# gam0022/hanamaru-renderer

Hardware: AMD Instinct MI355X
Metric: Mpaths/sec at 1920x1080x1024spp (rtcamp6 scene); achieved GB/s in BVH traversal (higher is better)
Workload: dtype f32

## Files before the change

hanamaru-renderer_amd/csrc/device_scene.h:

```cpp
#pragma once
#include <math.h>
#include <stdint.h>

#if defined(__HIPCC__)
#define HD __host__ __device__ __forceinline__
#else
#define HD inline
#endif

namespace hr {

struct alignas(16) f4 { float x, y, z, w; };

struct alignas(16) Node {
    float nearx, neary, farx, fary;
    float nearz, farz;
    uint32_t a;
    uint32_t b;
};
HD void node_set_box(Node &n, const float *mn, const float *mx, int octant) {
    n.nearx = (octant & 1) ? mx[0] : mn[0]; n.farx = (octant & 1) ? mn[0] : mx[0];
    n.neary = (octant & 2) ? mx[1] : mn[1]; n.fary = (octant & 2) ? mn[1] : mx[1];
    n.nearz = (octant & 4) ? mx[2] : mn[2]; n.farz = (octant & 4) ? mn[2] : mx[2];
}
// ... 156 lines not shown
    return B;
}
HD uint32_t gov_producer_prio(int32_t level, uint32_t init_prio) { return level <= 0 ? (init_prio | init_prio << 2) : level == 1 ? init_prio : 0u; }

struct RenderParams {
    uint32_t width, height;
    uint32_t tiles_x, tiles_y;
    uint32_t sampling_begin, stride, num_k;
    uint32_t adv_den;
    uint32_t leaf_den;
    uint32_t pad[3];
    uint32_t trace_boost;
    uint32_t node_unroll;
    uint32_t kchunk;
    uint32_t ovf_cap;
    uint32_t rr_start;
    uint32_t gov_slot;
    uint32_t nee_cull_off;
    uint32_t tail_div;
    uint32_t wg_budget;
    GovDev *gov;
    uint64_t rec_lo_off;
    uint32_t org_x, org_y, reg_w, reg_h;
};
HD uint32_t rp_reg_w(const RenderParams &rp) { return rp.reg_w ? rp.reg_w : rp.width; }
HD uint32_t rp_reg_h(const RenderParams &rp) { return rp.reg_h ? rp.reg_h : rp.height; }
HD bool rp_in_region(const RenderParams &rp, uint32_t px, uint32_t py) { return px < rp_reg_w(rp) && py < rp_reg_h(rp); }

HD void tile_lane_pixel(const RenderParams &rp, uint32_t tile, uint32_t j, uint32_t &px, uint32_t &py, uint32_t &sub) {
    uint32_t tx = tile % rp.tiles_x, ty = tile / rp.tiles_x;
    uint32_t pix = j >> 2;
    sub = j & 3u;
    px = tx * 4u + (pix & 3u);
    py = ty * 4u + (pix >> 2);
}
HD void tile_lane_frame_pixel(const RenderParams &rp, uint32_t tile, uint32_t j, uint32_t &px, uint32_t &py, uint32_t &sub) {
    tile_lane_pixel(rp, tile, j, px, py, sub);
    px += rp.org_x;
    py += rp.org_y;
}

static const int ISAAC_TAIL = 64;
static const int REC_FLOATS = 32;
static const int REC_DRAWS = 28;
static const int REC_HEAD = 28;
static const int LENS_FAST = 5;
// ... 14 lines not shown
```

hanamaru-renderer_amd/csrc/hr_api.hip:

```cpp
#include <hip/hip_runtime.h>

#include <cmath>
#include <cstdarg>
#include <cstdio>
#include <cstring>
#include <string>
#include <vector>

#include "bvh_build.h"
#include "device_scene.h"
#include "flatten.h"
#include "gpu_bvh.h"
#include "hanamaru_hip.h"
#include "hanamaru_hip_debug.h"
#include "hr_comm.h"
#include "isaac_core.h"
#include "post_core.h"
#include "pt_core.h"

using namespace hr;


static thread_local std::string g_err;
static int fail(int code, const char *fmt, ...) {
    char buf[1024];
    va_list ap;
    va_start(ap, fmt);
    vsnprintf(buf, sizeof buf, fmt, ap);
    va_end(ap);
    g_err = buf;
    return code;
}
#define HIP_TRY(expr)                                                                                         \
    do {                                                                                                      \
        hipError_t e_ = (expr);                                                                               \
        if (e_ != hipSuccess) return fail(HR_ERR_DEVICE, "%s failed: %s (%s:%d)", #expr, hipGetErrorString(e_), __FILE__, __LINE__); \
    } while (0)
// ... 41 lines not shown
    uint64_t batch_counter = 0;
    Counters *d_counters = nullptr;
    uint32_t *d_tile_counter = nullptr;
    bool counters = false;
    uint32_t batch = 0;
    uint32_t adv_den = 2, leaf_den = 2;
    int min_waves = 5;
    uint32_t trace_wgs = 6;
    uint32_t tail_div = 16;
    uint32_t trace_grid = 0, trace_budget = 0;
    uint32_t node_unroll = 2;
    uint32_t kchunk = 0;
    int trace_boost = -1;
    GovDev *gov = nullptr;
    bool quant_nodes = true;
    int max_leaf = 4;
    double split_ratio = -1.0;
    int bvh_builder = -1;
    int builder_in_use = 0;
    double bvh_build_ms = 0;
    uint64_t max_tail_bytes = 20ull << 30;
    int seed_mode = 2;
    int seed_prof = 0;
    uint32_t seed_prio = 3;
    uint32_t nee_cull = 7;
    uint32_t rr_start = 0;
    uint32_t ploc_top = hr::lbvh::PLOC_TOP_CLUSTERS;
    int trace_mode = 0;
    int trace_mode_opt = -1;
    int precise_opt = -1;
    bool precise = false;
    bool wf_has_prec = false;
    WfQueues wf{};
    void *wf_block = nullptr;
    uint32_t wf_adv_den = 2, wf_trav_wgs = 8, wf_shade_wgs = 8;
    int debug_skip = 0;
    std::vector<EventPair> seed_events, trace_events, post_events, debug_events;
    double seed_ms = 0, trace_ms = 0, post_ms = 0, debug_ms = 0;
    uint64_t seed_launches = 0, trace_launches = 0, debug_launches = 0;
    uint64_t paths_rendered = 0;
    std::vector<std::pair<uint64_t, hipEvent_t>> markers;
    uint64_t next_ticket = 1;
};

#include <map>
#include <mutex>
// ... 176 lines not shown
    HIP_TRY(hipStreamCreateWithFlags(&c->own_stream, hipStreamNonBlocking));
    HIP_TRY(hipStreamCreateWithFlags(&c->seed_stream, hipStreamNonBlocking));
    c->stream = c->own_stream;
    for (int i = 0; i < 2; i++) {
        HIP_TRY(hipEventCreateWithFlags(&c->seed_done[i], hipEventDisableTiming));
        HIP_TRY(hipEventCreateWithFlags(&c->trace_done[i], hipEventDisableTiming));
    }
    HIP_TRY(hipMalloc((void **)&c->d_counters, sizeof(Counters)));
    HIP_TRY(hipMemset(c->d_counters, 0, sizeof(Counters)));
    HIP_TRY(hipMalloc((void **)&c->d_tile_counter, 2 * sizeof(uint32_t)));
    HIP_TRY(hipMalloc((void **)&c->gov, sizeof(GovDev)));
    { int grc = govern_reset(c); if (grc) return grc; }
    HIP_TRY(hipFuncSetAttribute((const void *)seed_isaac64_kernel, hipFuncAttributeMaxDynamicSharedMemorySize, (int)SEED_LDS_BYTES));
HIP_TRY(hipFuncSetAttribute((const void *)seed_pc_kernel<8>, hipFuncAttributeMaxDynamicSharedMemorySize, (int)SEED_LDS_BYTES));
    HIP_TRY(hipFuncSetAttribute((const void *)seed_pc_kernel<12>, hipFuncAttributeMaxDynamicSharedMemorySize, (int)SEED_LDS_BYTES));
    HIP_TRY(hipFuncSetAttribute((const void *)seed_pc_kernel<16>, hipFuncAttributeMaxDynamicSharedMemorySize, (int)SEED_LDS_BYTES));
    HIP_TRY(hipFuncSetAttribute((const void *)seed_pc_kernel<20>, hipFuncAttributeMaxDynamicSharedMemorySize, (int)SEED_LDS_BYTES));
    HIP_TRY(hipFuncSetAttribute((const void *)seed_pc_kernel<24>, hipFuncAttributeMaxDynamicSharedMemorySize, (int)SEED_LDS_BYTES));
    HIP_TRY(hipFuncSetAttribute((const void *)seed_pc_kernel<28>, hipFuncAttributeMaxDynamicSharedMemorySize, (int)SEED_LDS_BYTES));
    HIP_TRY(hipFuncSetAttribute((const void *)seed_pc_kernel<16, true>, hipFuncAttributeMaxDynamicSharedMemorySize, (int)SEED_LDS_BYTES));
    HIP_TRY(hipFuncSetAttribute((const void *)seed_pc_kernel<20, true>, hipFuncAttributeMaxDynamicSharedMemorySize, (int)SEED_LDS_BYTES));
    HIP_TRY(hipFuncSetAttribute((const void *)seed_seg_kernel<false>, hipFuncAttributeMaxDynamicSharedMemorySize, (int)SEED_LDS_BYTES));
    HIP_TRY(hipFuncSetAttribute((const void *)seed_seg_kernel<true>, hipFuncAttributeMaxDynamicSharedMemorySize, (int)SEED_LDS_BYTES));
#if defined(HR_EXPERIMENTS)
    HIP_TRY(hipFuncSetAttribute((const void *)seed_w5_kernel<false>, hipFuncAttributeMaxDynamicSharedMemorySize, (int)SEED_LDS_BYTES));
    HIP_TRY(hipFuncSetAttribute((const void *)seed_w5_kernel<true>, hipFuncAttributeMaxDynamicSharedMemorySize, (int)SEED_LDS_BYTES));
    HIP_TRY(hipFuncSetAttribute((const void *)seed_ps_kernel<0>, hipFuncAttributeMaxDynamicSharedMemorySize, (int)SEED_LDS_BYTES));
    HIP_TRY(hipFuncSetAttribute((const void *)seed_ps_kernel<1>, hipFuncAttributeMaxDynamicSharedMemorySize, (int)SEED_LDS_BYTES));
    HIP_TRY(hipFuncSetAttribute((const void *)seed_ps_kernel<2>, hipFuncAttributeMaxDynamicSharedMemorySize, (int)SEED_LDS_BYTES));
    HIP_TRY(hipFuncSetAttribute((const void *)seed_ps_kernel<3>, hipFuncAttributeMaxDynamicSharedMemorySize, (int)SEED_LDS_BYTES));
#endif
    HIP_TRY(hipFuncSetAttribute((const void *)seed_debug_kernel, hipFuncAttributeMaxDynamicSharedMemorySize, 256 * 64 * 8));
    {
        const void *trace_variants[] = {(const void *)trace_kernel<false, 5, true>, (const void *)trace_kernel<false, 5, false>, (const void *)trace_kernel<false, 4, true>,
                                        (const void *)trace_kernel<false, 6, true>, (const void *)trace_kernel<true, 3, true>, (const void *)trace_kernel<true, 3, false>,
                                        (const void *)trace_kernel<false, 5, true, true>, (const void *)trace_kernel<false, 5, false, true>,
                                        (const void *)trace_kernel<true, 3, true, true>, (const void *)trace_kernel<true, 3, false, true>,
                                        (const void *)trace_kernel<false, 3, true, false, true>, (const void *)trace_kernel<false, 3, false, false, true>,
                                        (const void *)trace_kernel<false, 4, true, false, false, true>, (const void *)trace_kernel<false, 4, false, false, false, true>};
        for (const void *f : trace_variants) {
            hipFuncAttributes fa;
            HIP_TRY(hipFuncGetAttributes(&fa, f));
            if (fa.sharedSizeBytes != 0) return fail(HR_ERR_DEVICE, "build error: a trace kernel variant uses %zu bytes of LDS (it must use none to run beside the seed kernel)", (size_t)fa.sharedSizeBytes);
        }
    }
    HIP_TRY(hipMalloc((void **)&c->ovf_win, (size_t)c->num_cus * 2 * SEED_WIN_WORDS * sizeof(u64)));
    return HR_OK;
}

int hr_destroy(hr_ctx *c) {
    if (!c) return HR_OK;
    (void)hipSetDevice(c->device);
    (void)hipDeviceSynchronize();
    unbind_accumulator(c);
    free_scene(c);
    for (auto *ev : {&c->seed_events, &c->trace_events, &c->post_events, &c->debug_events})
        for (auto &e : *ev) { (void)hipEventDestroy(e.a); (void)hipEventDestroy(e.b); }
    for (auto &m : c->markers) (void)hipEventDestroy(m.second);
    if (c->accum_own) (void)hipFree(c->accum_own);
    for (int i = 0; i < 2; i++) {
        if (c->recs[i]) (void)hipFree(c->recs[i]);
        if (c->seed_done[i]) (void)hipEventDestroy(c->seed_done[i]);
        if (c->trace_done[i]) (void)hipEventDestroy(c->trace_done[i]);
    }
    if (c->ring) (void)hipFree(c->ring);
    if (c->wf_block) (void)hipFree(c->wf_block);
    if (c->ovf) (void)hipFree(c->ovf);
    if (c->ovf_win) (void)hipFree(c->ovf_win);
    if (c->d_counters) (void)hipFree(c->d_counters);
    if (c->d_tile_counter) (void)hipFree(c->d_tile_counter);
    if (c->gov) (void)hipFree(c->gov);
    if (c->post_tmp) (void)hipFree(c->post_tmp);
    if (c->d_rgb8) (void)hipFree(c->d_rgb8);
    if (c->accum_total) (void)hipFree(c->accum_total);
    if (c->comm && hrcomm::api().CommDestroy) (void)hrcomm::api().CommDestroy(c->comm);
    for (hr_ctx *p : c->same_device_peers) if (p != c) { p->same_device_peers.clear(); p->comm_world = 0; p->total_valid = false; p->comm_path = HR_COMM_NONE; p->allreduces = 0; }
    if (c->own_stream) (void)hipStreamDestroy(c->own_stream);
    if (c->seed_stream) (void)hipStreamDestroy(c->seed_stream);
    delete c;
    return HR_OK;
}

static int build_bvh_on_device(hr_ctx *c, const HostScene &hs, const Tri *tris_in) {
    using namespace lbvh;
    Scene &d = c->dsc;
    Prims p{};
    p.tris = tris_in; p.num_tris = d.num_tris; p.spheres = d.spheres; p.num_spheres = d.num_spheres; p.cuboids = d.cuboids; p.num_cuboids = d.num_cuboids;
    p.ref_tri = nullptr; p.ref_box = nullptr;
// ... 444 lines not shown
        HIP_TRY(mark());
#define HR_LAUNCH_SHADE(C, P, L) hipLaunchKernelGGL((wf_shade_kernel<C, P, L>), gs, b, 0, st, c->dsc, rp, c->recs[slot], wq, step, c->d_counters, plog)
        if (plog) { if (c->precise) HR_LAUNCH_SHADE(false, true, true); else HR_LAUNCH_SHADE(false, false, true); }
        else if (c->counters) { if (c->precise) HR_LAUNCH_SHADE(true, true, false); else HR_LAUNCH_SHADE(true, false, false); }
        else if (c->precise) HR_LAUNCH_SHADE(false, true, false);
        else HR_LAUNCH_SHADE(false, false, false);
#undef HR_LAUNCH_SHADE
        HIP_TRY(mark());
    }
    HIP_TRY(hipGetLastError());
    return HR_OK;
}

static int launch_seed(hr_ctx *c, const RenderParams &rp, int slot, hipStream_t st) {
    uint64_t paths = (uint64_t)rp.tiles_x * rp.tiles_y * rp.num_k * 64u;
    uint32_t grid = (uint32_t)std::min<uint64_t>((paths + SEED_COLS - 1) / SEED_COLS, (uint64_t)c->num_cus);
    EventPair ev{nullptr, nullptr};
    HIP_TRY(hipEventCreate(&ev.a));
    HIP_TRY(hipEventCreate(&ev.b));
    HIP_TRY(hipEventRecord(ev.a, st));
    if (c->debug_skip & 2) {
    } else if (c->seed_mode == 2) {
        if (!c->ring) HIP_TRY(hipMalloc((void **)&c->ring, (size_t)c->num_cus * SEED_RING_WORDS_MAX * sizeof(u64)));
#define HR_LAUNCH_SEG(P, L) hipLaunchKernelGGL((seed_seg_kernel<P, L>), dim3(grid), dim3(256), SEED_LDS_BYTES, st, rp, c->dsc.cam.lens_shape, c->ring, c->recs[slot], c->ovf, c->ovf_win, c->d_counters)
        if (rp.rec_lo_off) { if (c->seed_prof) HR_LAUNCH_SEG(true, true); else HR_LAUNCH_SEG(false, true); }
        else if (c->seed_prof) HR_LAUNCH_SEG(true, false);
        else HR_LAUNCH_SEG(false, false);
#undef HR_LAUNCH_SEG
#if defined(HR_EXPERIMENTS)
    } else if (c->seed_mode == 4) {
        if (!c->ring) HIP_TRY(hipMalloc((void **)&c->ring, (size_t)c->num_cus * SEED_RING_WORDS_MAX * sizeof(u64)));
        if (c->seed_prof) hipLaunchKernelGGL((seed_w5_kernel<true>), dim3(grid), dim3(320), SEED_LDS_BYTES, st, rp, c->dsc.cam.lens_shape, c->ring, c->recs[slot], c->ovf, c->ovf_win, c->d_counters);
        else hipLaunchKernelGGL((seed_w5_kernel<false>), dim3(grid), dim3(320), SEED_LDS_BYTES, st, rp, c->dsc.cam.lens_shape, c->ring, c->recs[slot], c->ovf, c->ovf_win, c->d_counters);
    } else if (c->seed_mode == 3) {
        if (!c->ring) HIP_TRY(hipMalloc((void **)&c->ring, (size_t)c->num_cus * SEED_RING_WORDS_MAX * sizeof(u64)));
#define HR_LAUNCH_PS(P) hipLaunchKernelGGL(seed_ps_kernel<P>, dim3(grid), dim3(256), SEED_LDS_BYTES, st, rp, c->dsc.cam.lens_shape, c->ring, c->recs[slot], c->ovf, c->ovf_win, c->d_counters)
        switch (c->seed_prof) { case 1: HR_LAUNCH_PS(1); break; case 2: HR_LAUNCH_PS(2); break; case 3: HR_LAUNCH_PS(3); break; default: HR_LAUNCH_PS(0); break; }
#undef HR_LAUNCH_PS
#endif
    } else if (c->seed_mode == 1) {
        if (!c->ring) HIP_TRY(hipMalloc((void **)&c->ring, (size_t)c->num_cus * SEED_RING_WORDS_MAX * sizeof(u64)));
#define HR_LAUNCH_PC(HEAD) hipLaunchKernelGGL(seed_pc_kernel<HEAD>, dim3(grid), dim3(256), SEED_LDS_BYTES, st, rp, c->dsc.cam.lens_shape, c->ring, c->recs[slot], c->ovf, c->ovf_win, c->d_counters)
        if (c->seed_prof && c->seed_split == 20) hipLaunchKernelGGL((seed_pc_kernel<20, true>), dim3(grid), dim3(256), SEED_LDS_BYTES, st, rp, c->dsc.cam.lens_shape, c->ring, c->recs[slot], c->ovf, c->ovf_win, c->d_counters);
        else if (c->seed_prof) hipLaunchKernelGGL((seed_pc_kernel<16, true>), dim3(grid), dim3(256), SEED_LDS_BYTES, st, rp, c->dsc.cam.lens_shape, c->ring, c->recs[slot], c->ovf, c->ovf_win, c->d_counters);
        else switch (c->seed_split) {
            case 8: HR_LAUNCH_PC(8); break;
            case 12: HR_LAUNCH_PC(12); break;
            case 20: HR_LAUNCH_PC(20); break;
            case 24: HR_LAUNCH_PC(24); break;
            case 28: HR_LAUNCH_PC(28); break;
            default: HR_LAUNCH_PC(16); break;
// ... 546 lines not shown
        return HR_OK;
    }
    if (k == "init_prio") {
        if (value < 0 || value > 3) return fail(HR_ERR_INVALID, "init_prio must be in [0,3]");
        c->init_prio = (uint32_t)value;
        return HR_OK;
    }
    if (k == "seed_split") {
        if (value != 8 && value != 12 && value != 16 && value != 20 && value != 24 && value != 28) return fail(HR_ERR_INVALID, "seed_split must be 8, 12, 16, 20, 24 or 28");
        c->seed_split = (int)value;
        return HR_OK;
    }
    if (k == "seed_mode") {
        if (value != 0 && value != 1 && value != 2 && value != 3 && value != 4) return fail(HR_ERR_INVALID, "seed_mode must be 4 (five-wave four-run kernel), 3 (phase-shifted four-run kernel), 2 (three-run kernel), 1 (producer / consumer kernel with a state ring) or 0 (fused kernel)");
#if !defined(HR_EXPERIMENTS)
        if (value >= 3) return fail(HR_ERR_UNSUPPORTED, "seed_mode %d is a measured experiment (slower than the default): build with `make EXPERIMENTS=1` to have it", (int)value);
#endif
        int rc = sync_all(c);
        if (rc) return rc;
        c->seed_mode = (int)value;
        return HR_OK;
    }
    if (k == "seed_prof") { c->seed_prof = (int)value; return HR_OK; }
    if (k == "ploc_top") {
        if (value < 1 || value > (1 << 16)) return fail(HR_ERR_INVALID, "ploc_top must be in [1,65536]");
        c->ploc_top = (uint32_t)value;
        return HR_OK;
    }
    if (k == "trace_mode") {
        if (value != -1 && value != 0 && value != 1) return fail(HR_ERR_INVALID, "trace_mode must be -1 (automatic), 0 (megakernel) or 1 (split: traversal kernel + shading kernel)");
        int rc = sync_all(c);
        if (rc) return rc;
        c->trace_mode_opt = (int)value;
        return govern_reset(c);
    }
    if (k == "draw_residuals") { if (value != 0 && value != 1) return fail(HR_ERR_INVALID, "draw_residuals must be 0 or 1"); c->draw_residuals = (int)value; return HR_OK; }
    if (k == "wf_adv_den") { if (value < 0 || value > 64) return fail(HR_ERR_INVALID, "wf_adv_den must be in [0,64]"); c->wf_adv_den = (uint32_t)value; return HR_OK; }
    if (k == "wf_trav_wgs") { if (value < 1 || value > 16) return fail(HR_ERR_INVALID, "wf_trav_wgs must be in [1,16]"); c->wf_trav_wgs = (uint32_t)value; return HR_OK; }
    if (k == "wf_shade_wgs") { if (value < 1 || value > 16) return fail(HR_ERR_INVALID, "wf_shade_wgs must be in [1,16]"); c->wf_shade_wgs = (uint32_t)value; return HR_OK; }
    if (k == "debug_skip") { c->debug_skip = (int)value; return HR_OK; }
    if (k == "nee_cull") { c->nee_cull = (uint32_t)value & 7u; return HR_OK; }
    return fail(HR_ERR_INVALID, "unknown debug option '%s'", key);
}

int hr_debug_draws(hr_ctx *c, uint32_t sampling, uint32_t first_path, uint32_t num_paths, uint32_t window, uint64_t *host_out) {
    if (!c || !host_out || !num_paths) return fail(HR_ERR_INVALID, "hr_debug_draws: bad argument");
// ... 41 lines not shown
    }
    for (uint32_t t = 0; t < tiles; t++)
        for (uint32_t j = 0; j < 64; j++) {
            uint32_t tx = t % rp.tiles_x, ty = t / rp.tiles_x, pix = j >> 2, sub = j & 3;
            uint32_t px = tx * 4 + (pix & 3), py = ty * 4 + (pix >> 2);
            if (px >= c->W || py >= c->H) continue;
            const float *rec = &h[(size_t)t * REC_ITEM_FLOATS];
            const uint32_t lb = j * 4u;
            uint32_t a = float_as_uint(rec[rec_slot(lb, REC_HEAD)]);
            float *o = &host_out[(((size_t)py * c->W + px) * 4 + sub) * DRAWS_PER_PATH];
            if (residuals) {
                const float *rl = &lo[(size_t)t * REC_ITEM_FLOATS];
                for (uint32_t d = 0; d < (uint32_t)DRAWS_PER_PATH; d++) o[d] = rl[rec_slot(lb, 2 * a + d)];
                continue;
            }
            o[0] = rec[rec_slot(lb, REC_HEAD + 1)];
            o[1] = rec[rec_slot(lb, REC_HEAD + 2)];
            for (uint32_t d = 2; d < (uint32_t)DRAWS_PER_PATH; d++) o[d] = rec[rec_slot(lb, 2 * a + d)];
        }
    return drain_events(c);
}
int hr_debug_path_draws(hr_ctx *c, uint32_t sampling, float *host_out) { return path_draws_out(c, sampling, host_out, false, "hr_debug_path_draws"); }
int hr_debug_path_draw_residuals(hr_ctx *c, uint32_t sampling, float *host_out) { return path_draws_out(c, sampling, host_out, true, "hr_debug_path_draw_residuals"); }

int hr_debug_path_log(hr_ctx *c, uint32_t sampling, uint32_t *host_out) {
    if (!c || !host_out) return fail(HR_ERR_INVALID, "hr_debug_path_log: bad argument");
    if (has_region(c)) return fail(HR_ERR_UNSUPPORTED, "hr_debug_path_log: not while a region is set (hr_set_region)");
    if (!c->W) return fail(HR_ERR_NO_TARGET, "hr_debug_path_log: hr_set_resolution not called");
    if (!c->have_scene) return fail(HR_ERR_NO_SCENE, "hr_debug_path_log: no scene uploaded");
    HIP_TRY(hipSetDevice(c->device));
    int rc = sync_all(c);
    if (rc) return rc;
    RenderParams rp{};
    rp.width = c->W; rp.height = c->H; rp.tiles_x = (c->W + 3) / 4; rp.tiles_y = (c->H + 3) / 4;
    rp.sampling_begin = sampling; rp.stride = 1; rp.num_k = 1;
    rp.adv_den = c->adv_den; rp.leaf_den = c->leaf_den; rp.node_unroll = c->node_unroll; rp.kchunk = c->kchunk;
    rp.pad[0] = c->seed_prio;
    rp.nee_cull_off = ~c->nee_cull & 7u;
    const uint32_t tiles = rp.tiles_x * rp.tiles_y;
    if ((rc = ensure_draws(c, tiles))) return rc;
    rp.rec_lo_off = rec_lo_off(c);
    if ((rc = ensure_ovf(c, (uint64_t)tiles * 64u))) return rc;
    rp.ovf_cap = c->ovf_cap;
    if ((rc = launch_seed(c, rp, 0, c->stream))) return rc;
    const size_t words = (size_t)c->W * c->H * 4u * 8u;
    uint32_t *d_log = nullptr;
// ... 140 lines not shown
```

hanamaru-renderer_amd/csrc/seed_kernels.h:

```cpp
#pragma once
#include <hip/hip_runtime.h>

#include "device_scene.h"
#include "isaac_core.h"

using namespace hr;


__device__ __forceinline__ uint32_t lds_addr(const void *p) { return (uint32_t)(size_t)(const __attribute__((address_space(3))) void *)p; }
__device__ __forceinline__ u64 lds_load64(uint32_t a) { return *(const __attribute__((address_space(3))) u64 *)(size_t)a; }

static const int SEED_COLS = 80;
static const int SEED_WAVES = 2, SEED_LANES = SEED_COLS / SEED_WAVES;
__device__ __forceinline__ uint32_t seed_gov_begin(const RenderParams &rp, bool stamp) {
    if (!rp.gov) return rp.pad[1];
    const int32_t lvl = __hip_atomic_load(&rp.gov->level, __ATOMIC_RELAXED, __HIP_MEMORY_SCOPE_AGENT);
    if (stamp) {
        atomicMin(&rp.gov->t0[0][rp.gov_slot], (unsigned long long)__builtin_amdgcn_s_memrealtime());
        if (blockIdx.x == 0) rp.gov->lvl[0][rp.gov_slot] = (uint32_t)lvl;
    }
    return gov_producer_prio(lvl, rp.pad[1] & 3u);
}
__device__ __forceinline__ void seed_gov_end(const RenderParams &rp, bool stamp) {
    if (rp.gov && stamp) atomicMax(&rp.gov->t1[0][rp.gov_slot], (unsigned long long)__builtin_amdgcn_s_memrealtime());
// ... 347 lines not shown
    SegLane l;
    if (lane < (uint32_t)SEED_LANES) { l.col = lane; l.run = consumer ? 2u : 0u; l.on = true; }
    else if (consumer) { l.col = lane - (uint32_t)SEED_LANES; l.run = 1u; l.on = true; }
    else { l.col = lane - 16u; l.run = 1u; l.on = lane < 56u; if (!l.on) l.col = (uint32_t)SEED_LANES - 1u; }
    return l;
}
struct SegRegs {
    typedef u64 u64x2_t __attribute__((ext_vector_type(2)));
    u64x2_t v[8];
    __device__ __forceinline__ void load(const u64 *ring_wg, uint64_t g, uint32_t half, const SegLane &l) {
        const u64 *regs = ring_wg + (g & (SEED_RING_GROUPS - 1)) * SegLayout::GROUP_WORDS + half * SegLayout::HALF_WORDS + (size_t)l.run * SegLayout::STATE_WORDS + (size_t)l.col * 2u;
#pragma unroll
        for (int q = 0; q < 8; q++) v[q] = __builtin_nontemporal_load(reinterpret_cast<const u64x2_t *>(regs + q * (2 * SEED_LANES)));
    }
    __device__ __forceinline__ void run(unsigned char *lds_half, const SegLane &l) const {
        u64 st16[16];
#pragma unroll
        for (int q = 0; q < 8; q++) { st16[2 * q] = v[q].x; st16[2 * q + 1] = v[q].y; }
        const uint32_t first = l.run == 0u ? 0u : l.run == 1u ? (uint32_t)SEG_B1 : (uint32_t)SEG_B2;
        LdsHalfMem m{reinterpret_cast<u64 *>(lds_half) + l.col + (size_t)first * 8u * SEED_LANES};
        if (l.on) isaac_init_run<SEG_NBLK>(m, st16);
    }
};
template <bool PROF, bool LO>
__device__ __forceinline__ void seed_seg_consumer(const RenderParams &rp, int lens_shape, const PcRange &r, unsigned char *smem, uint32_t lane, uint32_t half,
                                                  float *__restrict__ recs, uint32_t *__restrict__ ovf, u64 *__restrict__ win, Counters *cnt) {
    uint32_t *ovf_list = ovf + (size_t)(blockIdx.x * 2u + half) * rp.ovf_cap;
    uint32_t ovf_count = 0;
    unsigned long long pc[8] = {0, 0, 0, 0, 0, 0, 0, 0}, tm = 0;
#define HR_STAMP(i) do { if (PROF) { unsigned long long now_ = __builtin_readcyclecounter(); pc[i] += now_ - tm; tm = now_; } } while (0)
    const SegLane sl = seg_lane(true, lane);
    SegRegs regs;
    const uint32_t colr = lane < (uint32_t)SEED_LANES ? lane : 0u;
    unsigned char *lds_half = smem + (size_t)half * SEED_LDS_HALF_BYTES;
    LdsHalfMem m{reinterpret_cast<u64 *>(lds_half) + colr};
    const uint64_t n_groups = r.G1 - r.G0;
    __syncthreads();
    for (uint64_t it = 1; it <= n_groups; it++) {
        if (PROF) tm = __builtin_readcyclecounter();
        const uint64_t g = r.G0 + it - 1;
        if (it == 1) regs.load(r.ring_wg, g, half, sl);
        const uint64_t pid = g * SEED_COLS + half * SEED_LANES + colr;
        const bool in_range = pid < r.paths;
        const uint32_t item = (uint32_t)((in_range ? pid : r.paths - 1) >> 6), j = (uint32_t)((in_range ? pid : r.paths - 1) & 63u);
        uint32_t tile = item / rp.num_k;
        uint32_t px, py, sub;
        tile_lane_frame_pixel(rp, tile, j, px, py, sub);
        const bool valid = in_range && px < rp.width && py < rp.height;
        HR_STAMP(0);
        if (PROF) { __builtin_amdgcn_s_waitcnt(0x0F70); HR_STAMP(1); }
        regs.run(lds_half, sl);
        HR_STAMP(2);
        __syncthreads();
        HR_STAMP(3);
        if (it < n_groups) regs.load(r.ring_wg, r.G0 + it, half, sl);
        RecStore rs(recs, pid, rp.rec_lo_off);
        RecordTail<RecStore, LO> lt(rs, lens_shape);
        if (lane < (uint32_t)SEED_LANES) {
            isaac_round<REC_DRAWS>(m, lt);
            lt.finish();
        }
        HR_STAMP(4);
        ovf_note(lane < (uint32_t)SEED_LANES && valid && lt.overflow(), pid, ovf_list, ovf_count, rp.ovf_cap);
        HR_STAMP(5);
        if (PROF) pc[7]++;
        __syncthreads();
        HR_STAMP(6);
    }
#undef HR_STAMP
    if (PROF && lane == 0)
        for (int i = 0; i < 8; i++) atomicAdd(&cnt->seed_phase[i], pc[i]);
    const bool lane_on = lane < (uint32_t)SEED_LANES;
    seed_fixup_wave<LdsHalfMem, LO>(rp, lens_shape, m, colr, lane_on, ovf_list, ovf_count, win + (size_t)(blockIdx.x * 2u + half) * SEED_WIN_WORDS, recs, cnt);
}
__device__ __forceinline__ void seed_seg_producer(const RenderParams &rp, const PcRange &r, unsigned char *smem, uint32_t lane, uint32_t half, const uint32_t pprio) {
    const IsaacWarm warm = isaac_warm();
    const SegLane sl = seg_lane(false, lane);
    SegRegs regs;
    unsigned char *lds_half = smem + (size_t)half * SEED_LDS_HALF_BYTES;
    const uint64_t n_groups = r.G1 - r.G0;
    uint64_t frontier = r.first_path & ~63ull;
    auto ahead = [&](uint64_t upto) {
        const uint64_t need = upto * SEED_COLS;
        for (; frontier < need && frontier < r.end_path; frontier += 64) {
            if (((frontier >> 6) & 1u) != half) continue;
            const uint64_t pid0 = frontier + lane;
            const bool on = pid0 >= r.first_path && pid0 < r.end_path && !(rp.pad[2] & 4u);
            const uint64_t ppid = pid0 >= r.first_path && pid0 < r.end_path ? pid0 : r.end_path - 1;
            const uint32_t item = (uint32_t)(ppid >> 6), j = (uint32_t)(ppid & 63u);
            uint32_t tile = item / rp.num_k, k = item - tile * rp.num_k;
            uint32_t px, py, sub;
            tile_lane_frame_pixel(rp, tile, j, px, py, sub);
            bool pvalid = px < rp.width && py < rp.height;
            u64 s, t;
            path_seed_words(rp.width, rp.height, pvalid ? px : 0u, pvalid ? py : 0u, sub, s, t);
            const uint64_t g = ppid / SEED_COLS;
            const uint32_t c80 = (uint32_t)(ppid - g * SEED_COLS), hh = c80 >= (uint32_t)SEED_LANES ? 1u : 0u;
            SegStateOut out{r.ring_wg + (g & (SEED_RING_GROUPS - 1)) * SegLayout::GROUP_WORDS + hh * SegLayout::HALF_WORDS + (size_t)(c80 - hh * (uint32_t)SEED_LANES) * 2u};
            if (on) isaac_init_ahead<SEG_B1, SEG_B2>(out, warm, 8700304ULL, (u64)(rp.sampling_begin + k * rp.stride), s, t);
        }
        __builtin_amdgcn_s_waitcnt(0);
    };
    ahead(r.G0 + 2);
    __syncthreads();
    if (n_groups >= 1) regs.load(r.ring_wg, r.G0, half, sl);
    for (uint64_t it = 1; it <= n_groups; it++) {
        regs.run(lds_half, sl);
        __syncthreads();
        if (it < n_groups) regs.load(r.ring_wg, r.G0 + it, half, sl);
        if (((pprio >> 2) & 3u) != (pprio & 3u)) {
            const uint32_t pr = (it & 1u) ? (pprio >> 2) & 3u : pprio & 3u;
            if (pr == 0u) __builtin_amdgcn_s_setprio(0); else if (pr == 1u) __builtin_amdgcn_s_setprio(1); else if (pr == 2u) __builtin_amdgcn_s_setprio(2); else __builtin_amdgcn_s_setprio(3);
        }
        ahead(r.G0 + it + 2);
        __syncthreads();
    }
}
template <bool PROF = false, bool LO = false>
__global__ __launch_bounds__(256) void seed_seg_kernel(RenderParams rp, int lens_shape, u64 *__restrict__ ring, float *__restrict__ recs,
                                                       uint32_t *__restrict__ ovf, u64 *__restrict__ win, Counters *cnt) {
    extern __shared__ __align__(16) unsigned char smem[];
    const uint32_t lane = threadIdx.x & 63u, wave = threadIdx.x >> 6, half = wave & 1u;
    const bool consumer = wave < 2u;
    const uint32_t pprio = consumer ? 0u : seed_gov_begin(rp, wave == 2u && lane == 0u);
    const uint32_t prio = consumer ? rp.pad[0] : pprio & 3u;
    switch (prio) {
        case 0: break;
        case 1: __builtin_amdgcn_s_setprio(1); break;
        case 2: __builtin_amdgcn_s_setprio(2); break;
        default: __builtin_amdgcn_s_setprio(3); break;
    }
    PcRange r;
    r.paths = (uint64_t)rp.tiles_x * rp.tiles_y * rp.num_k * 64u;
    const uint64_t groups = (r.paths + SEED_COLS - 1) / SEED_COLS;
    r.G0 = groups * blockIdx.x / gridDim.x; r.G1 = groups * (blockIdx.x + 1) / gridDim.x;
    r.first_path = r.G0 * SEED_COLS; r.end_path = r.G1 * SEED_COLS < r.paths ? r.G1 * SEED_COLS : r.paths;
    r.ring_wg = ring + (size_t)blockIdx.x * SEED_RING_WORDS_MAX;
    if (consumer) seed_seg_consumer<PROF, LO>(rp, lens_shape, r, smem, lane, half, recs, ovf, win, cnt);
    else {
        seed_seg_producer(rp, r, smem, lane, half, pprio);
        seed_gov_end(rp, wave == 2u && lane == 0u);
    }
}

#if defined(HR_EXPERIMENTS)
static const int PS_NRUN = 4, PS_NBLK = 8, PS_P1BLK = 4;
struct PsLayout {
    static const size_t STATE_WORDS = (size_t)16 * SEED_LANES;
    static const size_t HALF_WORDS = PS_NRUN * STATE_WORDS;
    static const size_t GROUP_WORDS = 2 * HALF_WORDS;
};
static_assert(SEED_RING_GROUPS * PsLayout::GROUP_WORDS <= SEED_RING_WORDS_MAX, "the ring allocation of the producer / consumer kernel holds it");
struct PsStateOut {
    u64 *base;
    __device__ __forceinline__ void state(int k, u64 a, u64 b, u64 c, u64 d, u64 e, u64 f, u64 g, u64 h, u64 A, u64 B, u64 C, u64 D, u64 E, u64 F, u64 G, u64 H) {
        typedef u64 u64x2 __attribute__((ext_vector_type(2)));
        u64x2 *dst = reinterpret_cast<u64x2 *>(base + (size_t)k * PsLayout::STATE_WORDS);
        const u64x2 q[8] = {{a, b}, {c, d}, {e, f}, {g, h}, {A, B}, {C, D}, {E, F}, {G, H}};
#pragma unroll
        for (int j = 0; j < 8; j++) asm volatile("global_store_dwordx4 %0, %1, off sc1\n\ts_nop 1" : : "v"(dst + j * SEED_LANES), "v"(q[j]) : "memory");
    }
};
struct PsLane { uint32_t col, run; bool on; };
// ... 388 lines not shown
```

hanamaru-renderer_amd/python/hanamaru_amd/__init__.py:

```python
import ctypes as C
import os
import sys

import numpy as np

_HERE = os.path.dirname(os.path.abspath(__file__))
PKG_ROOT = os.path.normpath(os.path.join(_HERE, "..", ".."))
REPO_ROOT = os.path.normpath(os.path.join(PKG_ROOT, ".."))
ASSET_ROOT = os.path.join(REPO_ROOT, "assets")
HOST_LIB = os.path.join(PKG_ROOT, "libhanamaru_host.so")
HIP_LIB = os.path.join(PKG_ROOT, "libhanamaru_hip.so")

HR_OK = 0
HR_ERR_RNG_WINDOW = -5
DIFFUSE, SPECULAR, REFRACTION, GGX, GGX_REFRACTION = range(5)
SPHERE, CUBOID, MESH = range(3)


class Vec3(C.Structure):
    _fields_ = [("x", C.c_double), ("y", C.c_double), ("z", C.c_double)]

    def tuple(self):
        return (self.x, self.y, self.z)

# ... 109 lines not shown
        L.hr_get_region.argtypes = [C.c_void_p, C.POINTER(C.c_uint32)]
        L.hr_accumulator_device_ptr.argtypes = [C.c_void_p]
        L.hr_accumulator_device_ptr.restype = C.c_void_p
        L.hr_set_stream.argtypes = [C.c_void_p, C.c_void_p]
        L.hr_clear.argtypes = [C.c_void_p]
        L.hr_render.argtypes = [C.c_void_p, C.c_uint32, C.c_uint32, C.c_uint32]
        L.hr_synchronize.argtypes = [C.c_void_p]
        L.hr_mark.argtypes = [C.c_void_p, C.POINTER(C.c_uint64)]
        L.hr_wait.argtypes = [C.c_void_p, C.c_uint64]
        L.hr_render_debug.argtypes = [C.c_void_p, C.c_int]
        L.hr_read_accumulator.argtypes = [C.c_void_p, C.c_void_p]
        L.hr_write_accumulator.argtypes = [C.c_void_p, C.c_void_p]
        L.hr_resolve.argtypes = [C.c_void_p, C.c_uint32, C.c_void_p]
        L.hr_get_stats.argtypes = [C.c_void_p, C.POINTER(Stats)]
        L.hr_set_option.argtypes = [C.c_void_p, C.c_char_p, C.c_double]
        L.hr_set_debug_option.argtypes = [C.c_void_p, C.c_char_p, C.c_double]
        L.hr_debug_trace.argtypes = [C.c_void_p, C.c_uint32, C.c_void_p, C.c_void_p, C.c_void_p, C.c_void_p]
        L.hr_debug_draws.argtypes = [C.c_void_p, C.c_uint32, C.c_uint32, C.c_uint32, C.c_uint32, C.c_void_p]
        L.hr_debug_intersect.argtypes = [C.c_void_p, C.c_uint32, C.c_void_p, C.c_void_p, C.c_void_p]
        L.hr_debug_path_log.argtypes = [C.c_void_p, C.c_uint32, C.c_void_p]
        L.hr_debug_path_draws.argtypes = [C.c_void_p, C.c_uint32, C.c_void_p]
        L.hr_debug_path_draw_residuals.argtypes = [C.c_void_p, C.c_uint32, C.c_void_p]
        L.hr_debug_wf_profile.argtypes = [C.c_void_p, C.c_uint32, C.c_uint32, C.c_void_p, C.c_void_p]
        L.hr_comm_get_unique_id.argtypes = [C.c_void_p]
        L.hr_comm_init_rank.argtypes = [C.c_void_p, C.c_void_p, C.c_int, C.c_int]
        L.hr_comm_init_local.argtypes = [C.POINTER(C.c_void_p), C.c_int]
        L.hr_comm_destroy.argtypes = [C.c_void_p]
        L.hr_allreduce_accumulator.argtypes = [C.c_void_p]
        L.hr_allreduce_accumulators.argtypes = [C.POINTER(C.c_void_p), C.c_int]
        L.hr_total_device_ptr.argtypes = [C.c_void_p]
        L.hr_total_device_ptr.restype = C.c_void_p
        L.hr_comm_info.argtypes = [C.c_void_p, C.POINTER(CommInfo)]
        L.hr_accumulator_sum.argtypes = [C.c_void_p, C.c_int, C.POINTER(C.c_double)]
        _hip = L
    return _hip


COMM_ID_BYTES = 128


def comm_unique_id():
    L = hip_lib()
    buf = (C.c_char * COMM_ID_BYTES)()
    rc = L.hr_comm_get_unique_id(buf)
    if rc != 0:
        raise HipError(rc, L.hr_last_error().decode())
# ... 213 lines not shown
    def comm_info(self):
        ci = CommInfo()
        self._check(self.L.hr_comm_info(self._h, C.byref(ci)))
        return {"path": COMM_PATHS.get(ci.path, "?"), "nranks": int(ci.nranks), "rank": int(ci.rank), "device": int(ci.device),
                "rccl_version": int(ci.rccl_version), "allreduces": int(ci.allreduces)}

    def accumulator_sum(self, total=False):
        out = (C.c_double * 3)()
        self._check(self.L.hr_accumulator_sum(self._h, 1 if total else 0, out))
        return [float(out[0]), float(out[1]), float(out[2])]

    def debug_draws(self, sampling, first_path, num_paths, window):
        out = np.empty((num_paths, window), dtype=np.uint64)
        self._check(self.L.hr_debug_draws(self._h, sampling, first_path, num_paths, window, out.ctypes.data))
        return out

    def debug_path_log(self, sampling):
        raw = np.zeros((self.height, self.width, 4, 8), dtype=np.uint32)
        self._check(self.L.hr_debug_path_log(self._h, sampling, raw.ctypes.data))
        rad = raw[..., 0:3].copy().view(np.float32)
        ev = np.ascontiguousarray(raw[..., 4:7]).view(np.uint8).reshape(self.height, self.width, 4, 12)[..., :12]
        return rad, raw[..., 3].copy(), ev.copy(), raw[..., 7].copy()

    def debug_wf_profile(self, sampling=1, num_k=4):
        ms = np.zeros(21, dtype=np.float64)
        cn = np.zeros(22, dtype=np.uint32)
        self._check(self.L.hr_debug_wf_profile(self._h, sampling, num_k, ms.ctypes.data, cn.ctypes.data))
        return ms, cn.reshape(11, 2)

    def debug_intersect(self, rays):
        r = np.ascontiguousarray(rays, dtype=np.float32).reshape(-1, 6)
        out = np.empty((r.shape[0], 8), dtype=np.float32)
        el = np.empty((r.shape[0],), dtype=np.int32)
        self._check(self.L.hr_debug_intersect(self._h, r.shape[0], r.ctypes.data, out.ctypes.data, el.ctypes.data))
        return out, el

    def debug_trace(self, rays, shadow_len=None):
        r = np.ascontiguousarray(rays, dtype=np.float32).reshape(-1, 6)
        out = np.empty((r.shape[0], 8), dtype=np.float32)
        el = np.empty((r.shape[0],), dtype=np.int32)
        sl = None
        if shadow_len is not None:
            sl = np.ascontiguousarray(shadow_len, dtype=np.float32).reshape(-1)
            assert sl.shape[0] == r.shape[0]
        self._check(self.L.hr_debug_trace(self._h, r.shape[0], r.ctypes.data, sl.ctypes.data if sl is not None else None, out.ctypes.data, el.ctypes.data))
        return out, el
# ... 1 lines not shown
```

Measured before the change: 1361.

## Let seed workgroups claim path groups dynamically via a global atomic counter

```diff
diff --git a/hanamaru-renderer_amd/csrc/device_scene.h b/hanamaru-renderer_amd/csrc/device_scene.h
--- a/hanamaru-renderer_amd/csrc/device_scene.h
+++ b/hanamaru-renderer_amd/csrc/device_scene.h
@@ -202,6 +202,8 @@
     GovDev *gov;
     uint64_t rec_lo_off;
     uint32_t org_x, org_y, reg_w, reg_h;
+    uint32_t *claim_ctr;
+    uint32_t claim_base;
 };
 HD uint32_t rp_reg_w(const RenderParams &rp) { return rp.reg_w ? rp.reg_w : rp.width; }
 HD uint32_t rp_reg_h(const RenderParams &rp) { return rp.reg_h ? rp.reg_h : rp.height; }
diff --git a/hanamaru-renderer_amd/csrc/hr_api.hip b/hanamaru-renderer_amd/csrc/hr_api.hip
--- a/hanamaru-renderer_amd/csrc/hr_api.hip
+++ b/hanamaru-renderer_amd/csrc/hr_api.hip
@@ -13,6 +13,7 @@
 #include "gpu_bvh.h"
 #include "hanamaru_hip.h"
 #include "hanamaru_hip_debug.h"
+#include "hanamaru_hip_prof.h"
 #include "hr_comm.h"
 #include "isaac_core.h"
 #include "post_core.h"
@@ -100,6 +101,10 @@
     uint64_t max_tail_bytes = 20ull << 30;
     int seed_mode = 2;
     int seed_prof = 0;
+    int seed_claim = 1;
+    uint32_t *claim_ctr = nullptr;
+    uint32_t claim_next = 0;
+    uint32_t seed_grid = 0;
     uint32_t seed_prio = 3;
     uint32_t nee_cull = 7;
     uint32_t rr_start = 0;
@@ -322,6 +327,8 @@
     HIP_TRY(hipFuncSetAttribute((const void *)seed_pc_kernel<20, true>, hipFuncAttributeMaxDynamicSharedMemorySize, (int)SEED_LDS_BYTES));
     HIP_TRY(hipFuncSetAttribute((const void *)seed_seg_kernel<false>, hipFuncAttributeMaxDynamicSharedMemorySize, (int)SEED_LDS_BYTES));
     HIP_TRY(hipFuncSetAttribute((const void *)seed_seg_kernel<true>, hipFuncAttributeMaxDynamicSharedMemorySize, (int)SEED_LDS_BYTES));
+    HIP_TRY(hipFuncSetAttribute((const void *)seed_seg_kernel<false, false, false>, hipFuncAttributeMaxDynamicSharedMemorySize, (int)SEED_LDS_BYTES));
+    HIP_TRY(hipFuncSetAttribute((const void *)seed_seg_kernel<true, false, false>, hipFuncAttributeMaxDynamicSharedMemorySize, (int)SEED_LDS_BYTES));
 #if defined(HR_EXPERIMENTS)
     HIP_TRY(hipFuncSetAttribute((const void *)seed_w5_kernel<false>, hipFuncAttributeMaxDynamicSharedMemorySize, (int)SEED_LDS_BYTES));
     HIP_TRY(hipFuncSetAttribute((const void *)seed_w5_kernel<true>, hipFuncAttributeMaxDynamicSharedMemorySize, (int)SEED_LDS_BYTES));
@@ -364,6 +371,7 @@
         if (c->trace_done[i]) (void)hipEventDestroy(c->trace_done[i]);
     }
     if (c->ring) (void)hipFree(c->ring);
+    if (c->claim_ctr) (void)hipFree(c->claim_ctr);
     if (c->wf_block) (void)hipFree(c->wf_block);
     if (c->ovf) (void)hipFree(c->ovf);
     if (c->ovf_win) (void)hipFree(c->ovf_win);
@@ -854,11 +862,26 @@
     if (c->debug_skip & 2) {
     } else if (c->seed_mode == 2) {
         if (!c->ring) HIP_TRY(hipMalloc((void **)&c->ring, (size_t)c->num_cus * SEED_RING_WORDS_MAX * sizeof(u64)));
-#define HR_LAUNCH_SEG(P, L) hipLaunchKernelGGL((seed_seg_kernel<P, L>), dim3(grid), dim3(256), SEED_LDS_BYTES, st, rp, c->dsc.cam.lens_shape, c->ring, c->recs[slot], c->ovf, c->ovf_win, c->d_counters)
-        if (rp.rec_lo_off) { if (c->seed_prof) HR_LAUNCH_SEG(true, true); else HR_LAUNCH_SEG(false, true); }
-        else if (c->seed_prof) HR_LAUNCH_SEG(true, false);
-        else HR_LAUNCH_SEG(false, false);
+        if (!c->claim_ctr) {
+            HIP_TRY(hipMalloc((void **)&c->claim_ctr, sizeof(uint32_t)));
+            HIP_TRY(hipMemsetAsync(c->claim_ctr, 0, sizeof(uint32_t), st));
+            c->claim_next = 0;
+        }
+        RenderParams sp = rp;
+        sp.claim_ctr = c->claim_ctr;
+        sp.claim_base = c->claim_next;
+        const uint64_t claims = (paths + SEED_CLAIM_GROUPS * SEED_COLS - 1) / (SEED_CLAIM_GROUPS * SEED_COLS);
+        if (c->seed_claim) grid = (uint32_t)std::min<uint64_t>(claims, (uint64_t)c->num_cus);
+#define HR_LAUNCH_SEG(P, L, C) hipLaunchKernelGGL((seed_seg_kernel<P, L, C>), dim3(grid), dim3(256), SEED_LDS_BYTES, st, sp, c->dsc.cam.lens_shape, c->ring, c->recs[slot], c->ovf, c->ovf_win, c->d_counters)
+#define HR_LAUNCH_SEG_C(P, L) do { if (c->seed_claim) HR_LAUNCH_SEG(P, L, true); else HR_LAUNCH_SEG(P, L, false); } while (0)
+        if (rp.rec_lo_off) { if (c->seed_prof) HR_LAUNCH_SEG_C(true, true); else HR_LAUNCH_SEG_C(false, true); }
+        else if (c->seed_prof) HR_LAUNCH_SEG_C(true, false);
+        else HR_LAUNCH_SEG_C(false, false);
+#undef HR_LAUNCH_SEG_C
 #undef HR_LAUNCH_SEG
+        HIP_TRY(hipGetLastError());
+        if (c->seed_claim) c->claim_next += (uint32_t)claims;
+        c->seed_grid = grid;
 #if defined(HR_EXPERIMENTS)
     } else if (c->seed_mode == 4) {
         if (!c->ring) HIP_TRY(hipMalloc((void **)&c->ring, (size_t)c->num_cus * SEED_RING_WORDS_MAX * sizeof(u64)));
@@ -1451,6 +1474,11 @@
         return HR_OK;
     }
     if (k == "seed_prof") { c->seed_prof = (int)value; return HR_OK; }
+    if (k == "seed_claim") {
+        if (value != 0 && value != 1) return fail(HR_ERR_INVALID, "seed_claim must be 1 (workgroups claim groups dynamically) or 0 (fixed ranges)");
+        c->seed_claim = (int)value;
+        return HR_OK;
+    }
     if (k == "ploc_top") {
         if (value < 1 || value > (1 << 16)) return fail(HR_ERR_INVALID, "ploc_top must be in [1,65536]");
         c->ploc_top = (uint32_t)value;
@@ -1538,6 +1566,20 @@
 }
 int hr_debug_path_draws(hr_ctx *c, uint32_t sampling, float *host_out) { return path_draws_out(c, sampling, host_out, false, "hr_debug_path_draws"); }
 int hr_debug_path_draw_residuals(hr_ctx *c, uint32_t sampling, float *host_out) { return path_draws_out(c, sampling, host_out, true, "hr_debug_path_draw_residuals"); }
+
+int hr_debug_seed_timeline(hr_ctx *c, uint64_t *host_out, uint32_t capacity, uint32_t *workgroups) {
+    if (!c || !host_out || !workgroups) return fail(HR_ERR_INVALID, "hr_debug_seed_timeline: bad argument");
+    if (c->seed_mode != 2 || !c->seed_prof) return fail(HR_ERR_UNSUPPORTED, "hr_debug_seed_timeline: needs seed_mode 2 and seed_prof 1");
+    if (!c->ring || !c->seed_grid) return fail(HR_ERR_INVALID, "hr_debug_seed_timeline: no seed launch yet");
+    if (capacity < c->seed_grid) return fail(HR_ERR_INVALID, "hr_debug_seed_timeline: room for %u workgroups, the launch had %u", capacity, c->seed_grid);
+    HIP_TRY(hipSetDevice(c->device));
+    int rc = sync_all(c);
+    if (rc) return rc;
+    HIP_TRY(hipMemcpy2D(host_out, SEED_TL_WORDS * sizeof(u64), c->ring + SEED_TL_OFF, SEED_RING_WORDS_MAX * sizeof(u64), SEED_TL_WORDS * sizeof(u64), c->seed_grid,
+                        hipMemcpyDeviceToHost));
+    *workgroups = c->seed_grid;
+    return HR_OK;
+}
 
 int hr_debug_path_log(hr_ctx *c, uint32_t sampling, uint32_t *host_out) {
     if (!c || !host_out) return fail(HR_ERR_INVALID, "hr_debug_path_log: bad argument");
diff --git a/hanamaru-renderer_amd/csrc/seed_kernels.h b/hanamaru-renderer_amd/csrc/seed_kernels.h
--- a/hanamaru-renderer_amd/csrc/seed_kernels.h
+++ b/hanamaru-renderer_amd/csrc/seed_kernels.h
@@ -393,23 +393,45 @@
         if (l.on) isaac_init_run<SEG_NBLK>(m, st16);
     }
 };
-template <bool PROF, bool LO>
-__device__ __forceinline__ void seed_seg_consumer(const RenderParams &rp, int lens_shape, const PcRange &r, unsigned char *smem, uint32_t lane, uint32_t half,
+static const uint32_t SEED_CLAIM_GROUPS = 4;
+static_assert(SEED_CLAIM_GROUPS == (uint32_t)SEED_RING_GROUPS, "group g of a claim uses ring buffer g & 3 = its sequence number & 3");
+static_assert(SEED_CLAIM_GROUPS * SEED_COLS % 64 == 0, "a claim is whole chunks of the ahead pass");
+static const size_t SEED_CLAIM_OFF = SEED_RING_GROUPS * SegLayout::GROUP_WORDS;
+static const size_t SEED_TL_OFF = SEED_CLAIM_OFF + 4, SEED_TL_WORDS = 8;
+static_assert(SEED_TL_OFF + SEED_TL_WORDS <= SEED_RING_WORDS_MAX, "the ring allocation holds the claim slots and the stamps");
+__device__ __forceinline__ uint64_t seed_claim_load(const u64 *p) {
+    const u64 v = __hip_atomic_load(p, __ATOMIC_RELAXED, __HIP_MEMORY_SCOPE_AGENT);
+    return ((uint64_t)__builtin_amdgcn_readfirstlane((uint32_t)(v >> 32)) << 32) | __builtin_amdgcn_readfirstlane((uint32_t)v);
+}
+template <bool CLAIM>
+struct SegSeq {
+    uint64_t G0, G1;
+    u64 *slots;
+    uint64_t claim;
+    __device__ __forceinline__ uint64_t group(uint64_t s) {
+        if (!CLAIM) return G0 + s;
+        if ((s & 3u) == 0u) claim = seed_claim_load(slots + ((s >> 2) & 3u));
+        return claim * SEED_CLAIM_GROUPS + (s & 3u);
+    }
+};
+template <bool PROF, bool LO, bool CLAIM>
+__device__ __forceinline__ void seed_seg_consumer(const RenderParams &rp, int lens_shape, const PcRange &r, SegSeq<CLAIM> seq, unsigned char *smem, uint32_t lane, uint32_t half,
                                                   float *__restrict__ recs, uint32_t *__restrict__ ovf, u64 *__restrict__ win, Counters *cnt) {
     uint32_t *ovf_list = ovf + (size_t)(blockIdx.x * 2u + half) * rp.ovf_cap;
     uint32_t ovf_count = 0;
-    unsigned long long pc[8] = {0, 0, 0, 0, 0, 0, 0, 0}, tm = 0;
+    unsigned long long pc[8] = {0, 0, 0, 0, 0, 0, 0, 0}, tm = 0, t_entry = 0, t_a0 = 0;
 #define HR_STAMP(i) do { if (PROF) { unsigned long long now_ = __builtin_readcyclecounter(); pc[i] += now_ - tm; tm = now_; } } while (0)
+    if (PROF) t_entry = __builtin_amdgcn_s_memrealtime();
     const SegLane sl = seg_lane(true, lane);
     SegRegs regs;
     const uint32_t colr = lane < (uint32_t)SEED_LANES ? lane : 0u;
     unsigned char *lds_half = smem + (size_t)half * SEED_LDS_HALF_BYTES;
     LdsHalfMem m{reinterpret_cast<u64 *>(lds_half) + colr};
-    const uint64_t n_groups = r.G1 - r.G0;
+    uint64_t g = seq.G0;
     __syncthreads();
-    for (uint64_t it = 1; it <= n_groups; it++) {
+    if (PROF) t_a0 = __builtin_amdgcn_s_memrealtime();
+    for (uint64_t it = 1; g < seq.G1; it++) {
         if (PROF) tm = __builtin_readcyclecounter();
-        const uint64_t g = r.G0 + it - 1;
         if (it == 1) regs.load(r.ring_wg, g, half, sl);
         const uint64_t pid = g * SEED_COLS + half * SEED_LANES + colr;
         const bool in_range = pid < r.paths;
@@ -424,7 +446,8 @@
         HR_STAMP(2);
         __syncthreads();
         HR_STAMP(3);
-        if (it < n_groups) regs.load(r.ring_wg, r.G0 + it, half, sl);
+        const uint64_t g_next = seq.group(it);
+        if (g_next < seq.G1) regs.load(r.ring_wg, g_next, half, sl);
         RecStore rs(recs, pid, rp.rec_lo_off);
         RecordTail<RecStore, LO> lt(rs, lens_shape);
         if (lane < (uint32_t)SEED_LANES) {
@@ -437,57 +460,99 @@
         if (PROF) pc[7]++;
         __syncthreads();
         HR_STAMP(6);
+        g = g_next;
     }
 #undef HR_STAMP
+    const unsigned long long t_loop = PROF ? __builtin_amdgcn_s_memrealtime() : 0ull;
     if (PROF && lane == 0)
         for (int i = 0; i < 8; i++) atomicAdd(&cnt->seed_phase[i], pc[i]);
     const bool lane_on = lane < (uint32_t)SEED_LANES;
     seed_fixup_wave<LdsHalfMem, LO>(rp, lens_shape, m, colr, lane_on, ovf_list, ovf_count, win + (size_t)(blockIdx.x * 2u + half) * SEED_WIN_WORDS, recs, cnt);
-}
-__device__ __forceinline__ void seed_seg_producer(const RenderParams &rp, const PcRange &r, unsigned char *smem, uint32_t lane, uint32_t half, const uint32_t pprio) {
+    if (PROF && lane == 0) {
+        const unsigned long long t_fix = __builtin_amdgcn_s_memrealtime();
+        u64 *tl = r.ring_wg + SEED_TL_OFF;
+        tl[2 + half] = t_loop;
+        tl[4 + half] = t_fix;
+        if (half == 0u) {
+            tl[0] = t_entry;
+            tl[1] = t_a0;
+            tl[6] = pc[7];
+            tl[7] = ((u64)__builtin_amdgcn_s_getreg(20 | (31 << 11)) << 32) | __builtin_amdgcn_s_getreg(4 | (31 << 11));
+        }
+    }
+}
+template <bool CLAIM>
+__device__ __forceinline__ void seed_seg_producer(const RenderParams &rp, const PcRange &r, SegSeq<CLAIM> seq, unsigned char *smem, uint32_t lane, uint32_t half, const uint32_t pprio) {
     const IsaacWarm warm = isaac_warm();
     const SegLane sl = seg_lane(false, lane);
     SegRegs regs;
     unsigned char *lds_half = smem + (size_t)half * SEED_LDS_HALF_BYTES;
-    const uint64_t n_groups = r.G1 - r.G0;
+    auto chunk_states = [&](uint64_t chunk, uint64_t lo, uint64_t hi) {
+        const uint64_t pid0 = chunk + lane;
+        const bool on = pid0 >= lo && pid0 < hi && !(rp.pad[2] & 4u);
+        const uint64_t ppid = pid0 >= lo && pid0 < hi ? pid0 : hi - 1;
+        const uint32_t item = (uint32_t)(ppid >> 6), j = (uint32_t)(ppid & 63u);
+        uint32_t tile = item / rp.num_k, k = item - tile * rp.num_k;
+        uint32_t px, py, sub;
+        tile_lane_frame_pixel(rp, tile, j, px, py, sub);
+        bool pvalid = px < rp.width && py < rp.height;
+        u64 s, t;
+        path_seed_words(rp.width, rp.height, pvalid ? px : 0u, pvalid ? py : 0u, sub, s, t);
+        const uint64_t g = ppid / SEED_COLS;
+        const uint32_t c80 = (uint32_t)(ppid - g * SEED_COLS), hh = c80 >= (uint32_t)SEED_LANES ? 1u : 0u;
+        SegStateOut out{r.ring_wg + (g & (SEED_RING_GROUPS - 1)) * SegLayout::GROUP_WORDS + hh * SegLayout::HALF_WORDS + (size_t)(c80 - hh * (uint32_t)SEED_LANES) * 2u};
+        if (on) isaac_init_ahead<SEG_B1, SEG_B2>(out, warm, 8700304ULL, (u64)(rp.sampling_begin + k * rp.stride), s, t);
+    };
     uint64_t frontier = r.first_path & ~63ull;
+    uint64_t fq = 0, fclaim = seq.G0 / SEED_CLAIM_GROUPS, fv = 0;
+    uint32_t fc = 0;
     auto ahead = [&](uint64_t upto) {
-        const uint64_t need = upto * SEED_COLS;
-        for (; frontier < need && frontier < r.end_path; frontier += 64) {
-            if (((frontier >> 6) & 1u) != half) continue;
-            const uint64_t pid0 = frontier + lane;
-            const bool on = pid0 >= r.first_path && pid0 < r.end_path && !(rp.pad[2] & 4u);
-            const uint64_t ppid = pid0 >= r.first_path && pid0 < r.end_path ? pid0 : r.end_path - 1;
-            const uint32_t item = (uint32_t)(ppid >> 6), j = (uint32_t)(ppid & 63u);
-            uint32_t tile = item / rp.num_k, k = item - tile * rp.num_k;
-            uint32_t px, py, sub;
-            tile_lane_frame_pixel(rp, tile, j, px, py, sub);
-            bool pvalid = px < rp.width && py < rp.height;
-            u64 s, t;
-            path_seed_words(rp.width, rp.height, pvalid ? px : 0u, pvalid ? py : 0u, sub, s, t);
-            const uint64_t g = ppid / SEED_COLS;
-            const uint32_t c80 = (uint32_t)(ppid - g * SEED_COLS), hh = c80 >= (uint32_t)SEED_LANES ? 1u : 0u;
-            SegStateOut out{r.ring_wg + (g & (SEED_RING_GROUPS - 1)) * SegLayout::GROUP_WORDS + hh * SegLayout::HALF_WORDS + (size_t)(c80 - hh * (uint32_t)SEED_LANES) * 2u};
-            if (on) isaac_init_ahead<SEG_B1, SEG_B2>(out, warm, 8700304ULL, (u64)(rp.sampling_begin + k * rp.stride), s, t);
-        }
-        __builtin_amdgcn_s_waitcnt(0);
+        if (!CLAIM) {
+            const uint64_t need = (seq.G0 + upto) * SEED_COLS;
+            for (; frontier < need && frontier < r.end_path; frontier += 64) {
+                if (((frontier >> 6) & 1u) != half) continue;
+                chunk_states(frontier, r.first_path, r.end_path);
+            }
+        } else {
+            for (; fq * 64u < upto * SEED_COLS; fq++) {
+                if (fc == 0u && fq != 0u) fclaim = seed_claim_load(seq.slots + (fv & 3u));
+                const uint64_t chunk = fclaim * (SEED_CLAIM_GROUPS * SEED_COLS) + fc * 64u;
+                if (chunk >= r.paths) break;
+                if (fc == 4u) { fc = 0u; fv++; } else fc++;
+                if ((fq & 1u) != half) continue;
+                chunk_states(chunk, chunk, r.paths);
+            }
+        }
     };
-    ahead(r.G0 + 2);
+    const bool claimer = CLAIM && half == 0u;
+    uint32_t claimed = 0;
+    ahead(2);
+    __builtin_amdgcn_s_waitcnt(0);
     __syncthreads();
-    if (n_groups >= 1) regs.load(r.ring_wg, r.G0, half, sl);
-    for (uint64_t it = 1; it <= n_groups; it++) {
+    uint64_t g = seq.G0;
+    if (g < seq.G1) regs.load(r.ring_wg, g, half, sl);
+    for (uint64_t it = 1; g < seq.G1; it++) {
         regs.run(lds_half, sl);
         __syncthreads();
-        if (it < n_groups) regs.load(r.ring_wg, r.G0 + it, half, sl);
+        const uint64_t g_next = seq.group(it);
+        if (g_next < seq.G1) regs.load(r.ring_wg, g_next, half, sl);
         if (((pprio >> 2) & 3u) != (pprio & 3u)) {
             const uint32_t pr = (it & 1u) ? (pprio >> 2) & 3u : pprio & 3u;
             if (pr == 0u) __builtin_amdgcn_s_setprio(0); else if (pr == 1u) __builtin_amdgcn_s_setprio(1); else if (pr == 2u) __builtin_amdgcn_s_setprio(2); else __builtin_amdgcn_s_setprio(3);
         }
-        ahead(r.G0 + it + 2);
-        __syncthreads();
-    }
-}
-template <bool PROF = false, bool LO = false>
+        const bool claim_now = claimer && (it & 3u) == 1u;
+        if (claim_now && lane == 0u) claimed = atomicAdd(rp.claim_ctr, 1u);
+        ahead(it + 2);
+        if (claim_now && lane == 0u) {
+            const u64 c = (u64)gridDim.x + (uint32_t)(claimed - rp.claim_base);
+            __hip_atomic_store(seq.slots + (((it + 3u) >> 2) & 3u), c, __ATOMIC_RELAXED, __HIP_MEMORY_SCOPE_AGENT);
+        }
+        __builtin_amdgcn_s_waitcnt(0);
+        __syncthreads();
+        g = g_next;
+    }
+}
+template <bool PROF = false, bool LO = false, bool CLAIM = true>
 __global__ __launch_bounds__(256) void seed_seg_kernel(RenderParams rp, int lens_shape, u64 *__restrict__ ring, float *__restrict__ recs,
                                                        uint32_t *__restrict__ ovf, u64 *__restrict__ win, Counters *cnt) {
     extern __shared__ __align__(16) unsigned char smem[];
@@ -504,12 +569,20 @@
     PcRange r;
     r.paths = (uint64_t)rp.tiles_x * rp.tiles_y * rp.num_k * 64u;
     const uint64_t groups = (r.paths + SEED_COLS - 1) / SEED_COLS;
-    r.G0 = groups * blockIdx.x / gridDim.x; r.G1 = groups * (blockIdx.x + 1) / gridDim.x;
-    r.first_path = r.G0 * SEED_COLS; r.end_path = r.G1 * SEED_COLS < r.paths ? r.G1 * SEED_COLS : r.paths;
     r.ring_wg = ring + (size_t)blockIdx.x * SEED_RING_WORDS_MAX;
-    if (consumer) seed_seg_consumer<PROF, LO>(rp, lens_shape, r, smem, lane, half, recs, ovf, win, cnt);
+    SegSeq<CLAIM> seq;
+    seq.slots = r.ring_wg + SEED_CLAIM_OFF;
+    if (CLAIM) {
+        seq.G0 = (uint64_t)blockIdx.x * SEED_CLAIM_GROUPS; seq.G1 = groups; seq.claim = blockIdx.x;
+        r.G0 = seq.G0; r.G1 = groups; r.first_path = 0; r.end_path = r.paths;
+    } else {
+        r.G0 = groups * blockIdx.x / gridDim.x; r.G1 = groups * (blockIdx.x + 1) / gridDim.x;
+        r.first_path = r.G0 * SEED_COLS; r.end_path = r.G1 * SEED_COLS < r.paths ? r.G1 * SEED_COLS : r.paths;
+        seq.G0 = r.G0; seq.G1 = r.G1; seq.claim = 0;
+    }
+    if (consumer) seed_seg_consumer<PROF, LO, CLAIM>(rp, lens_shape, r, seq, smem, lane, half, recs, ovf, win, cnt);
     else {
-        seed_seg_producer(rp, r, smem, lane, half, pprio);
+        seed_seg_producer<CLAIM>(rp, r, seq, smem, lane, half, pprio);
         seed_gov_end(rp, wave == 2u && lane == 0u);
     }
 }
diff --git a/hanamaru-renderer_amd/python/hanamaru_amd/__init__.py b/hanamaru-renderer_amd/python/hanamaru_amd/__init__.py
--- a/hanamaru-renderer_amd/python/hanamaru_amd/__init__.py
+++ b/hanamaru-renderer_amd/python/hanamaru_amd/__init__.py
@@ -155,6 +155,7 @@
         L.hr_debug_path_draws.argtypes = [C.c_void_p, C.c_uint32, C.c_void_p]
         L.hr_debug_path_draw_residuals.argtypes = [C.c_void_p, C.c_uint32, C.c_void_p]
         L.hr_debug_wf_profile.argtypes = [C.c_void_p, C.c_uint32, C.c_uint32, C.c_void_p, C.c_void_p]
+        L.hr_debug_seed_timeline.argtypes = [C.c_void_p, C.c_void_p, C.c_uint32, C.POINTER(C.c_uint32)]
         L.hr_comm_get_unique_id.argtypes = [C.c_void_p]
         L.hr_comm_init_rank.argtypes = [C.c_void_p, C.c_void_p, C.c_int, C.c_int]
         L.hr_comm_init_local.argtypes = [C.POINTER(C.c_void_p), C.c_int]
@@ -414,6 +415,12 @@
         ev = np.ascontiguousarray(raw[..., 4:7]).view(np.uint8).reshape(self.height, self.width, 4, 12)[..., :12]
         return rad, raw[..., 3].copy(), ev.copy(), raw[..., 7].copy()
 
+    def debug_seed_timeline(self, capacity=1024):
+        out = np.zeros((capacity, 8), dtype=np.uint64)
+        n = C.c_uint32(0)
+        self._check(self.L.hr_debug_seed_timeline(self._h, out.ctypes.data, capacity, C.byref(n)))
+        return out[:n.value].copy()
+
     def debug_wf_profile(self, sampling=1, num_k=4):
         ms = np.zeros(21, dtype=np.float64)
         cn = np.zeros(22, dtype=np.uint32)
diff --git a/include/hanamaru_hip_prof.h b/include/hanamaru_hip_prof.h
--- /dev/null
+++ b/include/hanamaru_hip_prof.h
@@ -0,0 +1,15 @@
+#ifndef HANAMARU_HIP_PROF_H
+#define HANAMARU_HIP_PROF_H
+
+#include "hanamaru_hip.h"
+
+#ifdef __cplusplus
+extern "C" {
+#endif
+
+int hr_debug_seed_timeline(hr_ctx *ctx, uint64_t *host_out, uint32_t capacity, uint32_t *workgroups);
+
+#ifdef __cplusplus
+}
+#endif
+#endif
```

New measurement: 1366, median of 6. Within noise of the previous version (+0.4%).
